# tambetm/simple_dqn

Hardware: AMD Instinct MI355X
Metric: train_steps/sec (batch=32, 4x84x84 uint8) (higher is better)
Workload: dtype f32; 1 GPU; BASELINE.json configs[1]: Breakout shapes, batch_size=32, replay_size=1000000, num_actions=4, HIP Q-net + device replay gather fused into conv1; global_batch=32, parallelism=dp1 (independent learners, RCCL grad all-reduce), ring=HBM mirror

## Files before the change

### __graft_entry__.py

```python
import os
import subprocess
import sys

ROOT = os.path.dirname(os.path.abspath(__file__))
if ROOT not in sys.path:
    sys.path.insert(0, ROOT)


def build():
    csrc = os.path.join(ROOT, "simple_dqn_amd", "csrc")
    subprocess.check_call(["make", "-C", csrc, "-j4"])
    emul = os.path.join(ROOT, "tests", "emul")
    subprocess.check_call(["g++", "-O2", "-ffp-contract=off", "-shared", "-fPIC", "-o", os.path.join(emul, "libsdqn_emul.so"),
                           os.path.join(emul, "emul.cpp")])
    subprocess.check_call(["g++", "-O2", "-ffp-contract=off", "-shared", "-fPIC", "-o", os.path.join(emul, "libsdqn_emul_n16.so"),
                           os.path.join(emul, "emul_n16.cpp")])
    from oracle import build_ref
    build_ref.build()
    import simple_dqn_amd
    lib = simple_dqn_amd.load()
    assert lib.sdqn_version() >= 100
    return None


def smoke():
    import random
    import numpy as np
    import simple_dqn_amd as sd
    sys.path.insert(0, os.path.join(ROOT, "tests"))
    from util import make_args
    from oracle.dqn_numpy import OracleDQN, xavier_weights
    from oracle.replay_numpy import ReplayOracle, synthetic_fill

    if not os.path.exists(sd.lib_path()):
        build()
    A, B, size = 4, 32, 2000
    args = make_args(batch_size=B)
    mem, omem = sd.ReplayMemory(size, args), ReplayOracle(size, batch_size=B)
    synthetic_fill(mem, 0, num_actions=A)
    synthetic_fill(omem, 0, num_actions=A)
    mem.sync_mirror()
    net = sd.DeepQNetwork(A, args)
    ws = xavier_weights(A, 1)
    net.set_weights(ws, 0)
    net.update_target_network()
    o = OracleDQN(A, batch_size=B, weights=ws)
    random.seed(3)
    mb = [x.copy() for x in mem.getMinibatch()]
    random.seed(3)
    omb = omem.getMinibatch()
    for a, b in zip(mb, omb):
        assert np.array_equal(a, b), "replay gather mismatch"
    random.seed(3)
    net.train_from_memory(mem, 1)
    o.train(omb)
    q, qo = net.predict(mb[0]), o.predict(omb[0])
    err = float(np.abs(q - qo).max())
    assert err < 1e-4, "Q-value mismatch vs oracle: %g" % err
    print("smoke ok: Q max-abs err vs oracle %.3e, gather bit-exact, B=%d" % (err, B))
    return None


if __name__ == "__main__":
    build()
    if len(sys.argv) > 1 and sys.argv[1] == "smoke":
        smoke()
```

### simple_dqn_amd/csrc/gemm_engine.h

```cpp
#pragma once
#include <hip/hip_runtime.h>
#include <string.h>
#include "problems.h"
#include "n16_map.h"
#include "launch.h"

namespace sdqn {

typedef float f32x16 __attribute__((ext_vector_type(16)));

template <class P, class = void> struct a_elem { typedef float type; };
template <class P> struct a_elem<P, decltype((void)sizeof(typename P::AT))> { typedef typename P::AT type; };
template <class P, class = void> struct b_elem { typedef float type; };
template <class P> struct b_elem<P, decltype((void)sizeof(typename P::BT))> { typedef typename P::BT type; };
template <class P, class = void> struct stages_lds { static constexpr bool value = false; };
template <class P> struct stages_lds<P, decltype((void)P::STAGE_LDS)> { static constexpr bool value = P::STAGE_LDS; };
template <class P> struct Staged : P { static constexpr bool STAGE_LDS = true; };
template <class P, class = void> struct a_group4 { static constexpr bool value = false; };
template <class P> struct a_group4<P, decltype((void)P::A_GROUP4)> { static constexpr bool value = P::A_GROUP4; };
template <class P, class = void> struct uses_f16_wgrad { static constexpr bool value = false; };
template <class P> struct uses_f16_wgrad<P, decltype((void)P::F16_WGRAD)> { static constexpr bool value = P::F16_WGRAD; };
template <class P, class = void> struct has_preload { static constexpr bool value = false; };
template <class P> struct has_preload<P, decltype((void)P::PRELOAD)> { static constexpr bool value = P::PRELOAD; };
template <class P, class = void> struct has_preload_multi { static constexpr bool value = false; };
template <class P> struct has_preload_multi<P, decltype((void)P::PRELOAD_MULTI)> { static constexpr bool value = P::PRELOAD_MULTI; };
struct Lead { const void* p[5]; int B, s0, s1, ctl, r0, r1; };
static_assert(sizeof(Lead) == 64, "leading block: 16 dwords");
constexpr int LEAD_ON = 256;
#define SDQN_LEAD_PARAMS const void* lp0, const void* lp1, const void* lp2, const void* lp3, const void* lp4, int lB, int ls0, int ls1, int lctl, int lr0, int lr1
#define SDQN_LEAD_ARGS(L) (L).p[0], (L).p[1], (L).p[2], (L).p[3], (L).p[4], (L).B, (L).s0, (L).s1, (L).ctl, (L).r0, (L).r1
template <class T> struct lead_noref { typedef T type; };
template <class T> struct lead_noref<T&> { typedef T type; };
#define SDQN_LEAD_SET_(f, v) a.f = (typename lead_noref<decltype(a.f)>::type)(v)
#define SDQN_LEAD_FIELDS(f0, f1, f2, f3, f4, X) \
  static void lead_pack(const StepArgs& a, Lead& l) { l.p[0] = a.f0; l.p[1] = a.f1; l.p[2] = a.f2; l.p[3] = a.f3; l.p[4] = a.f4; l.s1 = a.X; } \
  __device__ static void lead_apply(StepArgs& a, const void* q0, const void* q1, const void* q2, const void* q3, const void* q4, int x) { \
    SDQN_LEAD_SET_(f0, q0); SDQN_LEAD_SET_(f1, q1); SDQN_LEAD_SET_(f2, q2); SDQN_LEAD_SET_(f3, q3); SDQN_LEAD_SET_(f4, q4); a.X = x; }
template <class P, class = void> struct has_lead { static constexpr bool value = false; };
template <class P> struct has_lead<P, decltype((void)P::LEAD)> { static constexpr bool value = P::LEAD; };
template <class P, class = void> struct has_lead_multi { static constexpr bool value = false; };
template <class P> struct has_lead_multi<P, decltype((void)P::LEAD_MULTI)> { static constexpr bool value = P::LEAD_MULTI; };
inline int lead_grid(const dim3& g) { return (int)(g.x | g.y << 16 | g.z << 24); }
inline bool lead_grid_fits(const dim3& g) { return g.x < 65536u && g.y < 256u && g.z < 128u; }
inline int lead_ctl(const StepArgs& a, bool on) {
  const bool fits = a.B < 128 && a.xcd_map >= 0 && a.xcd_map < 256 && a.nz >= 0 && a.nz < 16 && a.S4 >= 0 && a.S4 < 256;
  return (a.xcd_map & 255) | (on && fits ? LEAD_ON : 0) | ((a.nz & 15) << 12) | ((a.S4 & 255) << 16);
}
__device__ __forceinline__ void lead_scalars(StepArgs& a, int B, int ctl) { a.B = B; a.xcd_map = ctl & 255; a.nz = (ctl >> 12) & 15; a.S4 = (ctl >> 16) & 255; }
#define SDQN_LEAD_FWD lp0, lp1, lp2, lp3, lp4, lB, ls0, ls1, lctl, lr0, lr1
template <class P, class = void> struct uses_f16_mfma { static constexpr bool value = false; };
template <class P> struct uses_f16_mfma<P, decltype((void)P::F16_MFMA)> { static constexpr bool value = P::F16_MFMA; };
template <class P, class = void> struct n16_waves { static constexpr int value = 0; };
template <class P> struct n16_waves<P, decltype((void)P::N16_WAVES)> { static constexpr int value = P::N16_WAVES; };
template <class P, int NW> constexpr bool use_n16() {
  return NW > 1 && n16_waves<P>::value == NW && stages_lds<P>::value && !uses_f16_wgrad<P>::value && !uses_f16_mfma<P>::value;
}
template <class P, class = void> struct gated_store { static constexpr bool value = false; };
template <class P> struct gated_store<P, decltype((void)P::GATED)> { static constexpr bool value = P::GATED; };

constexpr int PANEL = 32 * 33;

__device__ __forceinline__ void wave_lds_sync() {
  __builtin_amdgcn_fence(__ATOMIC_RELEASE, "wavefront");
  __builtin_amdgcn_wave_barrier();
  __builtin_amdgcn_fence(__ATOMIC_ACQUIRE, "wavefront");
}


__device__ __forceinline__ int pick_half(int v, int s, bool hi) {
  const int lo = __builtin_amdgcn_readlane(v, s), up = __builtin_amdgcn_readlane(v, s + 4);
  return hi ? up : lo;
}
__device__ __forceinline__ int64_t pick_half(int64_t v, int s, bool hi) {
  const int i = s;
  const int l0 = __builtin_amdgcn_readlane((int)(v & 0xFFFFFFFF), i), l1 = __builtin_amdgcn_readlane((int)(v >> 32), i);
  const int u0 = __builtin_amdgcn_readlane((int)(v & 0xFFFFFFFF), i + 4), u1 = __builtin_amdgcn_readlane((int)(v >> 32), i + 4);
  const int64_t lo = ((int64_t)l1 << 32) | (uint32_t)l0, up = ((int64_t)u1 << 32) | (uint32_t)u0;
  return hi ? up : lo;
}

#ifdef SDQN_TIMING
__device__ unsigned long long* g_sdqn_dbg = nullptr;
#define SDQN_STAMP(ph) do { if (g_sdqn_dbg && threadIdx.x == 0) g_sdqn_dbg[((size_t)(blockIdx.x + gridDim.x * (blockIdx.y + gridDim.y * blockIdx.z)) * 8) + (ph)] = clock64(); } while (0)
__device__ unsigned long long* g_sdqn_wdbg = nullptr;
__device__ unsigned g_sdqn_wdbg_blocks = 0;
#define SDQN_WSTAMP_DECL unsigned long long wst_[4] = {0, 0, 0, 0}
#define SDQN_WSTAMP(ph) do { if (wst_[ph] == 0) wst_[ph] = clock64(); } while (0)
#define SDQN_WSTAMP_FLUSH do { unsigned long long* wd_ = g_sdqn_wdbg; if (wd_ && (threadIdx.x & 63) == 0) { \
  const size_t b_ = (size_t)(blockIdx.x + gridDim.x * (blockIdx.y + gridDim.y * blockIdx.z)); const unsigned nb_ = g_sdqn_wdbg_blocks; \
  if (b_ < nb_ && (threadIdx.x >> 6) < 16) { \
    for (int q_ = 0; q_ < 4; ++q_) wd_[(b_ * 16 + (threadIdx.x >> 6)) * 4 + q_] = wst_[q_]; \
    if (threadIdx.x == 0) { unsigned x_; asm volatile("s_getreg_b32 %0, hwreg(HW_REG_XCC_ID, 0, 4)" : "=s"(x_)); wd_[(size_t)nb_ * 64 + b_] = x_; } } } } while (0)
#else
#define SDQN_STAMP(ph) do {} while (0)
#define SDQN_WSTAMP_DECL do {} while (0)
#define SDQN_WSTAMP(ph) do {} while (0)
#define SDQN_WSTAMP_FLUSH do {} while (0)
#endif

template <class P, int NW>
constexpr int tile_lds() {
  return NW * PANEL * (stages_lds<P>::value && (P::A_K || P::B_K) ? ((P::A_K ? 1 : 0) + (P::B_K ? 1 : 0)) : 1);
}

__device__ __forceinline__ constexpr int kslot(int t, int h) { return 8 * (t >> 2) + 4 * h + (t & 3); }

template <class T>
__device__ __forceinline__ T ld_byte_off(const T* base, uint32_t byte_off) {
  return *reinterpret_cast<const T*>(reinterpret_cast<const char*>(base) + byte_off);
// ... 278 lines not shown
      pan_a[n16::pan_off(n16::PA, k, x)] = pra[j].x; pan_a[n16::pan_off(n16::PA, k + 1, x)] = pra[j].y;
      pan_a[n16::pan_off(n16::PA, k + 2, x)] = pra[j].z; pan_a[n16::pan_off(n16::PA, k + 3, x)] = pra[j].w;
    }
#pragma unroll
    for (int j = 0; j < 2; ++j) {
      const int x = n16::ld_x(lane, j), k = n16::ld_k(lane);
      pan_b[n16::pan_off(n16::PB, k, x)] = prb[j].x; pan_b[n16::pan_off(n16::PB, k + 1, x)] = prb[j].y;
      pan_b[n16::pan_off(n16::PB, k + 2, x)] = prb[j].z; pan_b[n16::pan_off(n16::PB, k + 3, x)] = prb[j].w;
    }
    if (kc + NW * 32 < kend) stage_load(kc + NW * 32);
    wave_lds_sync();
#pragma unroll
    for (int t = 0; t < 8; ++t) { fa0[t] = pan_a[n16::frag_a(lane, t, 0)]; fa1[t] = pan_a[n16::frag_a(lane, t, 1)]; fb[t] = pan_b[n16::frag_b(lane, t)]; }
    wave_lds_sync();
#ifdef SDQN_TIMING
    asm volatile("" :: "v"(fa0[0]), "v"(fa1[7]));
    SDQN_WSTAMP(2);
    asm volatile("" :: "v"(fb[0]), "v"(fb[7]));
    SDQN_WSTAMP(3);
    SDQN_STAMP(3);
#endif
#pragma unroll
    for (int t = 0; t < 8; ++t) {
      acc0 = __builtin_amdgcn_mfma_f32_16x16x4f32(fa0[t], fb[t], acc0, 0, 0, 0);
      acc1 = __builtin_amdgcn_mfma_f32_16x16x4f32(fa1[t], fb[t], acc1, 0, 0, 0);
    }
    kc += NW * 32;
  }

#ifdef SDQN_TIMING
  asm volatile("" :: "v"(acc0[0]), "v"(acc1[3]));
  SDQN_STAMP(4);
#endif
  if (wave < NW) {
    float* cw = smem + wave * n16::WAVE_LDS;
#pragma unroll
    for (int r = 0; r < 4; ++r) {
      cw[n16::comb_off(n16::acc_row(0, lane, r), n16::acc_col(lane))] = acc0[r];
      cw[n16::comb_off(n16::acc_row(1, lane, r), n16::acc_col(lane))] = acc1[r];
    }
  }
  __syncthreads();
  SDQN_STAMP(5);
  static_assert(NT >= n16::TM * n16::TN, "one thread per element of the tile");
  if (mine) {
    float v = smem[n16::comb_off(ml, nl)];
#pragma unroll
    for (int w = 1; w < NW; ++w) v += smem[w * n16::WAVE_LDS + n16::comb_off(ml, nl)];
    if constexpr (gated_store<P>::value) P::store_gated(a, z, ks, m0 + ml, n0 + nl, v, gate);
    else P::store(a, z, ks, m0 + ml, n0 + nl, v);
  }
  SDQN_STAMP(6);
  SDQN_WSTAMP_FLUSH;
}

template <class P, int NW, int NT>
__device__ __forceinline__ void gemm_tile_h(const StepArgs& a, int bx, int by, int bz, float* smem) {
  constexpr int WAVE_LDS = PANEL;
  typedef typename P::aoff_t aoff_t;
  const int lane = threadIdx.x & 63;
  const int wave = __builtin_amdgcn_readfirstlane(threadIdx.x >> 6);
  const int m0 = bx * 32, n0 = by * 32;
  int z, ks, kbeg, kend;
  P::ksplit(a, bz, z, ks, kbeg, kend);
  if (NW * 64 < NT && wave >= NW) kend = kbeg;
  const int M = P::M(a), N = P::N(a);
  const int i = lane & 31, h8 = (lane >> 5) * 8;
  const aoff_t arow = P::a_row(a, z, m0 + i < M ? m0 + i : M - 1);
  const int bcol = P::b_col(a, z, n0 + i < N ? n0 + i : N - 1);
  f32x16 acc;
#pragma unroll
  for (int r = 0; r < 16; ++r) acc[r] = 0.0f;
  for (int kc = kbeg + (wave < NW ? wave : 0) * 32; kc < kend; kc += NW * 32) {
    const half8 fa0 = P::a_load8(a, z, arow + P::a_col(a, z, kc + h8));
    const half8 fb0 = P::b_load8(a, z, bcol + P::b_row(a, z, kc + h8));
    const half8 fa1 = P::a_load8(a, z, arow + P::a_col(a, z, kc + 16 + h8));
    const half8 fb1 = P::b_load8(a, z, bcol + P::b_row(a, z, kc + 16 + h8));
    acc = __builtin_amdgcn_mfma_f32_32x32x16_f16(fa0, fb0, acc, 0, 0, 0);
    acc = __builtin_amdgcn_mfma_f32_32x32x16_f16(fa1, fb1, acc, 0, 0, 0);
  }
  if constexpr (NW > 1) {
    if (wave < NW) {
      float* cw = smem + wave * WAVE_LDS;
#pragma unroll
      for (int r = 0; r < 16; ++r) {
        const int row = (r & 3) + 8 * (r >> 2) + 4 * (lane >> 5);
        cw[row * 33 + (lane & 31)] = acc[r];
      }
    }
    __syncthreads();
    for (int e = threadIdx.x; e < 1024; e += NT) {
      const int ml = e >> 5, nl = e & 31;
      float v = smem[ml * 33 + nl];
#pragma unroll
      for (int w = 1; w < NW; ++w) v += smem[w * WAVE_LDS + ml * 33 + nl];
      if (m0 + ml < M && n0 + nl < N) P::store(a, z, ks, m0 + ml, n0 + nl, v);
    }
  } else {
#pragma unroll
    for (int r = 0; r < 16; ++r) {
      const int ml = (r & 3) + 8 * (r >> 2) + 4 * (lane >> 5), nl = lane & 31;
      if (m0 + ml < M && n0 + nl < N) P::store(a, z, ks, m0 + ml, n0 + nl, acc[r]);
    }
  }
}

// ... 67 lines not shown
    wave_lds_sync();
#pragma unroll
    for (int s = 0; s < 2; ++s) {
      half8 fa, fb;
#pragma unroll
      for (int j = 0; j < 8; ++j) fb[j] = sb[(16 * s + 8 * hb + j) * HW_PITCH + i];
      if constexpr (P::A_U8) {
#pragma unroll
        for (int g = 0; g < 2; ++g) {
          const int src = 16 * s + 4 * g;
          const int l0 = __builtin_amdgcn_readlane((int)(cv & 0xFFFFFFFF), src), l1 = __builtin_amdgcn_readlane((int)((int64_t)cv >> 32), src);
          const int u0 = __builtin_amdgcn_readlane((int)(cv & 0xFFFFFFFF), src + 8), u1 = __builtin_amdgcn_readlane((int)((int64_t)cv >> 32), src + 8);
          const int64_t lo = ((int64_t)l1 << 32) | (uint32_t)l0, up = ((int64_t)u1 << 32) | (uint32_t)u0;
          const int64_t c = hi ? up : lo;
          const bool ok = kcur + 16 * s + 8 * hb + 4 * g < kend;
          const f4 v = P::a_load_group4(a, z, arow_own + c);
          fa[4 * g] = ok ? (half_t)v.x : (half_t)0.0f; fa[4 * g + 1] = ok ? (half_t)v.y : (half_t)0.0f;
          fa[4 * g + 2] = ok ? (half_t)v.z : (half_t)0.0f; fa[4 * g + 3] = ok ? (half_t)v.w : (half_t)0.0f;
        }
      } else {
#pragma unroll
        for (int j = 0; j < 8; ++j) fa[j] = sa[(16 * s + 8 * hb + j) * HW_PITCH + i];
      }
      acc = __builtin_amdgcn_mfma_f32_32x32x16_f16(fa, fb, acc, 0, 0, 0);
    }
    wave_lds_sync();
  }

  if constexpr (NW > 1) {
    if (wave < NW) {
      float* cw = smem + wave * HW_WAVE_LDS;
#pragma unroll
      for (int r = 0; r < 16; ++r) cw[((r & 3) + 8 * (r >> 2) + 4 * hb) * 33 + i] = acc[r];
    }
    __syncthreads();
    for (int e = threadIdx.x; e < 1024; e += NT) {
      const int ml = e >> 5, nl = e & 31;
      float v = smem[ml * 33 + nl];
#pragma unroll
      for (int w = 1; w < NW; ++w) v += smem[w * HW_WAVE_LDS + ml * 33 + nl];
      if (m0 + ml < M && n0 + nl < N) P::store(a, z, ks, m0 + ml, n0 + nl, v);
    }
  } else {
    float v[16];
#pragma unroll
    for (int r = 0; r < 16; ++r) v[r] = acc[r];
    P::store16(a, z, ks, m0, n0, lane, M, N, v, epi);
  }
}

template <class P, int NW, int NT>
__device__ __forceinline__ void run_tile(const StepArgs& a, int bx, int by, int bz, float* smem) {
  if constexpr (use_n16<P, NW>()) gemm_tile_n16<P, NW, NT>(a, bx, by, bz, smem);
  else if constexpr (uses_f16_wgrad<P>::value) gemm_tile_hw<P, NW, NT>(a, bx, by, bz, smem);
  else if constexpr (uses_f16_mfma<P>::value) gemm_tile_h<P, NW, NT>(a, bx, by, bz, smem);
  else gemm_tile<P, NW, NT>(a, bx, by, bz, smem);
}
template <class P, int NW>
constexpr int tile_lds_any() {
  if constexpr (use_n16<P, NW>()) return NW * n16::WAVE_LDS;
  else if constexpr (uses_f16_wgrad<P>::value) return NW * HW_WAVE_LDS;
  else return uses_f16_mfma<P>::value ? NW * PANEL : tile_lds<P, NW>();
}
template <class P> constexpr int tile_m() { return 32; }
template <class P, int NW = 0> constexpr int tile_n() { return use_n16<P, NW>() ? n16::TN : 32; }


template <class P>
__device__ __forceinline__ void lead_take(StepArgs& a, int& gx, int& gy, int& gz, const StepArgs& a_, SDQN_LEAD_PARAMS) {
  (void)lr0; (void)lr1;
  if (lctl & LEAD_ON) { lead_scalars(a, lB, lctl); P::lead_apply(a, lp0, lp1, lp2, lp3, lp4, ls1); gx = ls0 & 0xFFFF; gy = (ls0 >> 16) & 255; gz = ls0 >> 24; }
  else { if constexpr (has_preload<P>::value) P::preload(a_, gridDim.x, gridDim.y, gridDim.z); gx = gridDim.x; gy = gridDim.y; gz = gridDim.z; }
}
template <class P, int NW>
__device__ __forceinline__ void gemm_kernel_body(const StepArgs& a, int gx, int gy, int gz, float* smem) {
  const int lin = blockIdx.x + gx * (blockIdx.y + gy * blockIdx.z);
  const int t = (a.xcd_map & 1) ? xcd_tile_id(lin, gx * gy * gz) : lin;
  const int bz = t / (gx * gy), r = t - bz * (gx * gy);
  run_tile<P, NW, NW * 64>(a, r % gx, r / gx, bz, smem);
}
template <class P, int NW>
__global__ void __launch_bounds__(NW * 64) gemm_kernel(SDQN_LEAD_PARAMS, const StepArgs a_) {
  __shared__ float smem[tile_lds_any<P, NW>()];
  (void)lr0; (void)lr1;
  if constexpr (has_lead<P>::value) {
    StepArgs a = a_;
    int gx, gy, gz;
    lead_take<P>(a, gx, gy, gz, a_, SDQN_LEAD_FWD);
    gemm_kernel_body<P, NW>(a, gx, gy, gz, smem);
  } else {
    if constexpr (has_preload<P>::value) P::preload(a_, gridDim.x, gridDim.y, gridDim.z);
    gemm_kernel_body<P, NW>(a_, gridDim.x, gridDim.y, gridDim.z, smem);
  }
}

struct MultiDims { int n[3]; int gx[3], gy[3]; };

template <class P, int NW, int NT>
__device__ __forceinline__ void multi_dispatch(const StepArgs& a, const MultiDims& d, int which, int local, float* smem) {
  static_assert(!use_n16<P, NW>(), "multi-problem launches size their tile grids for 32 x 32 tiles");
  if constexpr (NW == 1) {
    const int wave = __builtin_amdgcn_readfirstlane(threadIdx.x >> 6);
    const int t = local * (NT / 64) + wave;
    const int per_z = d.gx[which] * d.gy[which];
    if (t < a.f4w_count) {
      const int tile = a.f4w_first + t;
      const int bz = tile / per_z, r = tile - bz * per_z;
      run_tile<P, 1, 64>(a, r % d.gx[which], r / d.gx[which], bz, smem);
    }
  } else {
    const int per_z = d.gx[which] * d.gy[which];
    const int bz = local / per_z, r = local - bz * per_z;
    run_tile<P, NW, NT>(a, r % d.gx[which], r / d.gx[which], bz, smem);
  }
}

template <int NT, class P0, int NW0, class P1, int NW1, class P2, int NW2>
__device__ __forceinline__ void gemm_multi_body(const StepArgs& a, const MultiDims& d, float* smem) {
  const int b = blockIdx.x;
  const int xm = a.xcd_map;
  if (b < d.n[0]) multi_dispatch<P0, NW0, NT>(a, d, 0, (xm & 1) ? xcd_tile_id_range(b, 0, d.n[0]) : b, smem);
  else if (b < d.n[0] + d.n[1]) multi_dispatch<P1, NW1, NT>(a, d, 1, (xm & 2) ? xcd_tile_id_range(b, d.n[0], d.n[1]) : b - d.n[0], smem);
  else multi_dispatch<P2, NW2, NT>(a, d, 2, (xm & 4) ? xcd_tile_id_range(b, d.n[0] + d.n[1], d.n[2]) : b - d.n[0] - d.n[1], smem);
}
template <int NT, class P0, int NW0, class P1, int NW1, class P2, int NW2>
__global__ void __launch_bounds__(NT) gemm_multi_kernel(SDQN_LEAD_PARAMS, const StepArgs a_, const MultiDims d_) {
  constexpr int L0 = tile_lds_any<P0, NW0>() * (NW0 == 1 ? NT / 64 : 1), L1 = tile_lds_any<P1, NW1>() * (NW1 == 1 ? NT / 64 : 1),
                L2 = tile_lds_any<P2, NW2>() * (NW2 == 1 ? NT / 64 : 1);
  constexpr int L = L0 > L1 ? (L0 > L2 ? L0 : L2) : (L1 > L2 ? L1 : L2);
  __shared__ float smem[L];
  (void)lr0; (void)lr1;
  if constexpr (has_lead_multi<P1>::value) {
    StepArgs a = a_; MultiDims d = d_;
    if (lctl & LEAD_ON) {
      lead_scalars(a, lB, lctl); P1::lead_apply(a, lp0, lp1, lp2, lp3, lp4, ls1);
      d.n[0] = ls0 & 0xFFFF; d.n[1] = (int)((unsigned)ls0 >> 16);
      d.gx[0] = (P0::M(a) + tile_m<P0>() - 1) / tile_m<P0>(); d.gy[0] = (P0::N(a) + tile_n<P0>() - 1) / tile_n<P0>();
      d.gx[1] = (P1::M(a) + tile_m<P1>() - 1) / tile_m<P1>(); d.gy[1] = (P1::N(a) + tile_n<P1>() - 1) / tile_n<P1>();
      d.gx[2] = (P2::M(a) + tile_m<P2>() - 1) / tile_m<P2>(); d.gy[2] = (P2::N(a) + tile_n<P2>() - 1) / tile_n<P2>();
    } else { if constexpr (has_preload_multi<P1>::value) P1::preload_multi(a_, d_); }
    gemm_multi_body<NT, P0, NW0, P1, NW1, P2, NW2>(a, d, smem);
  } else {
    if constexpr (has_preload_multi<P1>::value) P1::preload_multi(a_, d_);
    gemm_multi_body<NT, P0, NW0, P1, NW1, P2, NW2>(a_, d_, smem);
  }
}

struct NoProblem {
  static constexpr bool A_K = false, B_K = false; typedef int aoff_t; struct Epi {};
  static constexpr bool A_REG = false, A_U8 = false, B_REG = false; static constexpr int A_LD = 0, B_LD = 0;
  SDQN_HD static const float* a_ptr(const StepArgs&, int) { return nullptr; }
  SDQN_HD static const float* b_ptr(const StepArgs&, int) { return nullptr; }
  SDQN_HD static int M(const StepArgs&) { return 0; }
  SDQN_HD static int N(const StepArgs&) { return 0; }
  SDQN_HD static int nbz(const StepArgs&) { return 0; }
  SDQN_HD static void ksplit(const StepArgs&, int, int& z, int& ks, int& kb, int& ke) { z = ks = kb = ke = 0; }
  SDQN_HD static int a_row(const StepArgs&, int, int) { return 0; }
  SDQN_HD static int a_col(const StepArgs&, int, int) { return 0; }
  SDQN_HD static float a_load(const StepArgs&, int, int) { return 0.f; }
  SDQN_HD static f4 a_load4(const StepArgs&, int, int) { f4 o; o.x = o.y = o.z = o.w = 0.f; return o; }
  SDQN_HD static f4 b_load4(const StepArgs&, int, int) { f4 o; o.x = o.y = o.z = o.w = 0.f; return o; }
  SDQN_HD static int b_row(const StepArgs&, int, int) { return 0; }
  SDQN_HD static int b_col(const StepArgs&, int, int) { return 0; }
  SDQN_HD static float b_load(const StepArgs&, int, int) { return 0.f; }
  SDQN_HD static void store(const StepArgs&, int, int, int, int, float) {}
  __device__ static void epi_begin(const StepArgs&, int, int, int, Epi&) {}
  __device__ static void store16(const StepArgs&, int, int, int, int, int, int, int, const float*, Epi&) {}
};

template <class P, int NW>
inline hipError_t launch_gemm(const StepArgs& a, hipStream_t stream) {
  dim3 grid((P::M(a) + tile_m<P>() - 1) / tile_m<P>(), (P::N(a) + tile_n<P, NW>() - 1) / tile_n<P, NW>(), P::nbz(a));
  Lead l; memset(&l, 0, sizeof l);
  if constexpr (has_lead<P>::value) {
    P::lead_pack(a, l); l.B = a.B; l.s0 = lead_grid(grid);
    l.ctl = lead_ctl(a, a.arg_preload && lead_grid_fits(grid));
  }
  SDQN_LAUNCH((gemm_kernel<P, NW>), grid, dim3(NW * 64), 0, stream, SDQN_LEAD_ARGS(l), a);
  return hipGetLastError();
}

template <int NT, class P, int NW>
inline void multi_fill(const StepArgs& a, MultiDims& d, int i) {
  d.gx[i] = (P::M(a) + tile_m<P>() - 1) / tile_m<P>(); d.gy[i] = (P::N(a) + tile_n<P>() - 1) / tile_n<P>();
  const int tiles = d.gx[i] * d.gy[i] * P::nbz(a);
  d.n[i] = NW == 1 ? (a.f4w_count + NT / 64 - 1) / (NT / 64) : tiles;
}
template <int NT, class P0, int NW0, class P1, int NW1, class P2, int NW2>
inline hipError_t launch_multi(const StepArgs& a, bool has1, bool has2, hipStream_t stream) {
  static_assert(NW0 * 64 <= NT && NW1 * 64 <= NT && NW2 * 64 <= NT, "waves per tile exceed the workgroup");
  MultiDims d; memset(&d, 0, sizeof d);
  multi_fill<NT, P0, NW0>(a, d, 0);
  if (has1) multi_fill<NT, P1, NW1>(a, d, 1);
  if (has2) multi_fill<NT, P2, NW2>(a, d, 2);
  if (d.n[0] + d.n[1] + d.n[2] == 0) return hipSuccess;
  Lead l; memset(&l, 0, sizeof l);
  if constexpr (has_lead_multi<P1>::value) {
    P1::lead_pack(a, l); l.B = a.B; l.s0 = (int)((unsigned)d.n[0] | (unsigned)d.n[1] << 16);
    l.ctl = lead_ctl(a, a.arg_preload && has1 && has2 && d.n[0] < 65536 && d.n[1] < 65536);
  }
  SDQN_LAUNCH((gemm_multi_kernel<NT, P0, NW0, P1, NW1, P2, NW2>), dim3(d.n[0] + d.n[1] + d.n[2]), dim3(NT), 0, stream, SDQN_LEAD_ARGS(l), a, d);
  return hipGetLastError();
}

}
```

### simple_dqn_amd/csrc/problems.h

```cpp
#pragma once
#include <stddef.h>
#include <stdint.h>
#include <math.h>

#if defined(__HIPCC__)
#define SDQN_HD __host__ __device__ inline
#else
#define SDQN_HD inline
#endif

namespace sdqn {

constexpr int H0 = 84, W0 = 84, C0 = 4;
constexpr int FRAME = H0 * W0;
constexpr int STATE = C0 * FRAME;
constexpr int ST1 = 4, P1 = 20, Q1 = 20, K1 = 32;
constexpr int ST2 = 2, P2 = 9, Q2 = 9, K2 = 64;
constexpr int P3 = 7, Q3 = 7, K3 = 64;
constexpr int PIX1 = P1 * Q1, PIX2 = P2 * Q2, PIX3 = P3 * Q3;
constexpr int CRS1 = 256, CRS2 = 512, CRS3 = 576;
constexpr int NFC = 512, NIN4 = PIX3 * K3;
constexpr int PD3 = 11, PD2 = 11;
constexpr int NW1 = CRS1 * K1, NW2 = CRS2 * K2, NW3 = CRS3 * K3, NW4 = NIN4 * NFC;
constexpr int OFF1 = 0, OFF2 = OFF1 + NW1, OFF3 = OFF2 + NW2, OFF4 = OFF3 + NW3, OFF5 = OFF4 + NW4;
// ... 192 lines not shown
}


SDQN_HD int64_t row1(const StepArgs& a, int z, int m) {
  int n = m / PIX1, pix = m - n * PIX1, p = pix / Q1, q = pix - p * Q1;
  return sbase(a, z, n) + (int64_t)(p * ST1) * W0 + q * ST1;
}
SDQN_HD int col1(int k) { int c = k >> 6, r = (k >> 3) & 7, s = k & 7; return c * FRAME + r * W0 + s; }
SDQN_HD int row2(const StepArgs& a, int z, int m) {
  int n = m / PIX2, pix = m - n * PIX2, p = pix / Q2, q = pix - p * Q2;
  return (((z * a.B + n) * P1 + p * ST2) * Q1 + q * ST2) * K1;
}
SDQN_HD int col2(int k) { int r = k >> 7, s = (k >> 5) & 3, c = k & 31; return (r * Q1 + s) * K1 + c; }
SDQN_HD int row3(const StepArgs& a, int z, int m) {
  int n = m / PIX3, pix = m - n * PIX3, p = pix / Q3, q = pix - p * Q3;
  return (((z * a.B + n) * P2 + p) * Q2 + q) * K2;
}
SDQN_HD int col3(int k) { int rs = k >> 6, c = k & 63, r = rs / 3, s = rs - r * 3; return (r * Q2 + s) * K2 + c; }
SDQN_HD int prow2(int m) {
  int n = m / PIX2, pix = m - n * PIX2, p = pix / Q2, q = pix - p * Q2;
  return ((n * PD2 + p + 1) * PD2 + q + 1) * K2;
}

struct Conv1Fwd {
  static constexpr bool A_K = true, B_K = false;
  typedef int64_t aoff_t;
  static constexpr bool A_REG = false, A_U8 = true, B_REG = true; static constexpr int A_LD = 0, B_LD = K1;
  SDQN_HD static const float* a_ptr(const StepArgs& a, int z) { (void)z; return (const float*)nullptr; }
  SDQN_HD static const float* b_ptr(const StepArgs& a, int z) { (void)z; return a.theta[wslot(z)] + OFF1; }
#if defined(__HIPCC__)
  struct Epi {};
  __device__ static void epi_begin(const StepArgs&, int, int, int, Epi&) {}
  __device__ static void store16(const StepArgs& a, int z, int ks, int m0, int n0, int lane, int M, int N, const float* v, Epi&);
#endif
  SDQN_HD static int M(const StepArgs& a) { return a.B * PIX1; }
  SDQN_HD static int N(const StepArgs&) { return K1; }
  SDQN_HD static int nbz(const StepArgs& a) { return a.nz; }
  SDQN_HD static void ksplit(const StepArgs&, int bz, int& z, int& ks, int& kb, int& ke) { z = bz; ks = 0; kb = 0; ke = CRS1; }
  SDQN_HD static aoff_t a_row(const StepArgs& a, int z, int m) { return row1(a, z, m); }
  SDQN_HD static aoff_t a_col(const StepArgs&, int, int k) { return col1(k); }
  SDQN_HD static float a_load(const StepArgs& a, int, aoff_t o) { return norm_u8(a.src[o]); }
  SDQN_HD static f4 a_load4(const StepArgs& a, int, aoff_t o) { return ld4_u8(a.src + o); }
  SDQN_HD static int b_row(const StepArgs&, int, int k) { return k * K1; }
  SDQN_HD static int b_col(const StepArgs&, int, int n) { return n; }
  SDQN_HD static float b_load(const StepArgs& a, int z, int o) { return a.theta[wslot(z)][OFF1 + o]; }
  SDQN_HD static f4 b_load4(const StepArgs& a, int z, int o) { return ld4(a.theta[wslot(z)] + OFF1 + o); }
  SDQN_HD static void store(const StepArgs& a, int z, int, int m, int n, float v) {
    a.a1[((int64_t)z * M(a) + m) * K1 + n] = fmaxf(v, 0.0f);
  }
};

struct Conv2Fwd {
  static constexpr bool A_K = true, B_K = false;
  typedef int aoff_t;
  static constexpr bool A_REG = false, A_U8 = false, B_REG = true; static constexpr int A_LD = 0, B_LD = K2;
  SDQN_HD static const float* a_ptr(const StepArgs& a, int z) { (void)z; return a.a1; }
  SDQN_HD static const float* b_ptr(const StepArgs& a, int z) { (void)z; return a.theta[wslot(z)] + OFF2; }
#if defined(__HIPCC__)
  struct Epi {};
  __device__ static void epi_begin(const StepArgs&, int, int, int, Epi&) {}
  __device__ static void store16(const StepArgs& a, int z, int ks, int m0, int n0, int lane, int M, int N, const float* v, Epi&);
#endif
  SDQN_HD static int M(const StepArgs& a) { return a.B * PIX2; }
  SDQN_HD static int N(const StepArgs&) { return K2; }
  SDQN_HD static int nbz(const StepArgs& a) { return a.nz; }
  SDQN_HD static void ksplit(const StepArgs&, int bz, int& z, int& ks, int& kb, int& ke) { z = bz; ks = 0; kb = 0; ke = CRS2; }
  SDQN_HD static aoff_t a_row(const StepArgs& a, int z, int m) { return row2(a, z, m); }
  SDQN_HD static aoff_t a_col(const StepArgs&, int, int k) { return col2(k); }
  SDQN_HD static float a_load(const StepArgs& a, int, aoff_t o) { return a.a1[o]; }
  SDQN_HD static f4 a_load4(const StepArgs& a, int, aoff_t o) { return ld4(a.a1 + o); }
  SDQN_HD static int b_row(const StepArgs&, int, int k) { return k * K2; }
  SDQN_HD static int b_col(const StepArgs&, int, int n) { return n; }
  SDQN_HD static float b_load(const StepArgs& a, int z, int o) { return a.theta[wslot(z)][OFF2 + o]; }
  SDQN_HD static f4 b_load4(const StepArgs& a, int z, int o) { return ld4(a.theta[wslot(z)] + OFF2 + o); }
  SDQN_HD static void store(const StepArgs& a, int z, int, int m, int n, float v) {
    a.a2[((int64_t)z * M(a) + m) * K2 + n] = fmaxf(v, 0.0f);
  }
};

struct Conv3Fwd {
  static constexpr bool A_K = true, B_K = false;
  typedef int aoff_t;
  static constexpr bool A_REG = false, A_U8 = false, B_REG = true; static constexpr int A_LD = 0, B_LD = K3;
  SDQN_HD static const float* a_ptr(const StepArgs& a, int z) { (void)z; return a.a2; }
  SDQN_HD static const float* b_ptr(const StepArgs& a, int z) { (void)z; return a.theta[wslot(z)] + OFF3; }
#if defined(__HIPCC__)
  struct Epi {};
  __device__ static void epi_begin(const StepArgs&, int, int, int, Epi&) {}
  __device__ static void store16(const StepArgs& a, int z, int ks, int m0, int n0, int lane, int M, int N, const float* v, Epi&);
#endif
  SDQN_HD static int M(const StepArgs& a) { return a.B * PIX3; }
  SDQN_HD static int N(const StepArgs&) { return K3; }
  SDQN_HD static int nbz(const StepArgs& a) { return a.nz; }
  SDQN_HD static void ksplit(const StepArgs&, int bz, int& z, int& ks, int& kb, int& ke) { z = bz; ks = 0; kb = 0; ke = CRS3; }
  SDQN_HD static aoff_t a_row(const StepArgs& a, int z, int m) { return row3(a, z, m); }
  SDQN_HD static aoff_t a_col(const StepArgs&, int, int k) { return col3(k); }
  SDQN_HD static float a_load(const StepArgs& a, int, aoff_t o) { return a.a2[o]; }
  SDQN_HD static f4 a_load4(const StepArgs& a, int, aoff_t o) { return ld4(a.a2 + o); }
  SDQN_HD static int b_row(const StepArgs&, int, int k) { return k * K3; }
  SDQN_HD static int b_col(const StepArgs&, int, int n) { return n; }
  SDQN_HD static float b_load(const StepArgs& a, int z, int o) { return a.theta[wslot(z)][OFF3 + o]; }
  SDQN_HD static f4 b_load4(const StepArgs& a, int z, int o) { return ld4(a.theta[wslot(z)] + OFF3 + o); }
  SDQN_HD static void store(const StepArgs& a, int z, int, int m, int n, float v) {
    a.a3[((int64_t)z * M(a) + m) * K3 + n] = fmaxf(v, 0.0f);
  }
};
// ... 265 lines not shown
struct Conv1Wgrad {
  static constexpr bool A_K = false, B_K = false;
  typedef int64_t aoff_t;
  static constexpr bool A_REG = false, A_U8 = true, B_REG = true; static constexpr int A_LD = 0, B_LD = K1;
  SDQN_HD static const float* a_ptr(const StepArgs& a, int z) { (void)z; return (const float*)nullptr; }
  SDQN_HD static const float* b_ptr(const StepArgs& a, int z) { (void)z; return a.d1; }
#if defined(__HIPCC__)
  struct Epi {};
  __device__ static void epi_begin(const StepArgs&, int, int, int, Epi&) {}
  __device__ static void store16(const StepArgs& a, int z, int ks, int m0, int n0, int lane, int M, int N, const float* v, Epi&);
#endif
  SDQN_HD static int Kt(const StepArgs& a) { return a.B * PIX1; }
  SDQN_HD static int M(const StepArgs&) { return CRS1; }
  SDQN_HD static int N(const StepArgs&) { return K1; }
  SDQN_HD static int nbz(const StepArgs& a) { return ceil_div(ceil_div(Kt(a), 32), a.tps1); }
  SDQN_HD static void ksplit(const StepArgs& a, int bz, int& z, int& ks, int& kb, int& ke) {
    z = 0; ks = bz; kb = bz * a.tps1 * 32; ke = kb + a.tps1 * 32; if (ke > Kt(a)) ke = Kt(a);
  }
  SDQN_HD static aoff_t a_row(const StepArgs&, int, int m) { return col1(m); }
  SDQN_HD static aoff_t a_col(const StepArgs& a, int, int k) { return row1(a, 0, k); }
  SDQN_HD static float a_load(const StepArgs& a, int, aoff_t o) { return norm_u8(a.src[o]); }
  SDQN_HD static f4 a_load4(const StepArgs& a, int, aoff_t o) { return ld4_u8(a.src + o); }
  static constexpr bool A_GROUP4 = true;
  SDQN_HD static f4 a_load_group4(const StepArgs& a, int, aoff_t o) { return ld4_u8_stride4(a.src + o); }
  SDQN_HD static int b_row(const StepArgs&, int, int k) { return k * K1; }
  SDQN_HD static int b_col(const StepArgs&, int, int n) { return n; }
  SDQN_HD static float b_load(const StepArgs& a, int, int o) { return a.d1[o]; }
  SDQN_HD static f4 b_load4(const StepArgs& a, int, int o) { return ld4(a.d1 + o); }
  SDQN_HD static void store(const StepArgs& a, int, int ks, int m, int n, float v) { a.slab1[(int64_t)ks * NW1 + m * K1 + n] = v; }
};

#if defined(__HIPCC__)
#define SDQN_STORE16_DEFAULT(P) __device__ inline void P::store16(const StepArgs& a, int z, int ks, int m0, int n0, int lane, int M, int N, const float* v, P::Epi&) { \
  _Pragma("unroll") for (int r = 0; r < 16; ++r) { const int ml = (r & 3) + 8 * (r >> 2) + 4 * (lane >> 5), nl = lane & 31; \
    if (m0 + ml < M && n0 + nl < N) P::store(a, z, ks, m0 + ml, n0 + nl, v[r]); } }
SDQN_STORE16_DEFAULT(Conv1Fwd)
SDQN_STORE16_DEFAULT(Conv2Fwd)
SDQN_STORE16_DEFAULT(Conv3Fwd)
SDQN_STORE16_DEFAULT(Fc4Fwd)
SDQN_STORE16_DEFAULT(Fc4Dgrad)
SDQN_STORE16_DEFAULT(Conv3Dgrad)
SDQN_STORE16_DEFAULT(Conv3Wgrad)
SDQN_STORE16_DEFAULT(Conv2Dgrad)
SDQN_STORE16_DEFAULT(Conv2Wgrad)
SDQN_STORE16_DEFAULT(Conv1Wgrad)
#endif

struct Conv1FwdRaw : Conv1Fwd {
  SDQN_HD static void store(const StepArgs& a, int z, int, int m, int n, float v) { a.a1[((int64_t)z * M(a) + m) * K1 + n] = v; }
#if defined(__HIPCC__)
  __device__ static void store16(const StepArgs& a, int z, int ks, int m0, int n0, int lane, int M, int N, const float* v, Epi&);
#endif
};
struct Conv2FwdRaw : Conv2Fwd {
  SDQN_HD static void store(const StepArgs& a, int z, int, int m, int n, float v) { a.a2[((int64_t)z * M(a) + m) * K2 + n] = v; }
#if defined(__HIPCC__)
  __device__ static void store16(const StepArgs& a, int z, int ks, int m0, int n0, int lane, int M, int N, const float* v, Epi&);
#endif
};
struct Conv3FwdRaw : Conv3Fwd {
  SDQN_HD static void store(const StepArgs& a, int z, int, int m, int n, float v) { a.a3[((int64_t)z * M(a) + m) * K3 + n] = v; }
#if defined(__HIPCC__)
  __device__ static void store16(const StepArgs& a, int z, int ks, int m0, int n0, int lane, int M, int N, const float* v, Epi&);
#endif
};
#if defined(__HIPCC__)
SDQN_STORE16_DEFAULT(Conv1FwdRaw)
SDQN_STORE16_DEFAULT(Conv2FwdRaw)
SDQN_STORE16_DEFAULT(Conv3FwdRaw)
#endif

inline int64_t neon_to_internal(int layer, int64_t row, int64_t col) {
  switch (layer) {
    case 0: return row * K1 + col;
    case 1: { int c = (int)(row / 16), rs = (int)(row % 16); return ((int64_t)rs * 32 + c) * K2 + col; }
    case 2: { int c = (int)(row / 9), rs = (int)(row % 9); return ((int64_t)rs * 64 + c) * K3 + col; }
    case 3: { int f = (int)(col / PIX3), pix = (int)(col % PIX3); return ((int64_t)pix * K3 + f) * NFC + row; }
    default: return row * NFC + col;
  }
}
inline void layer_dims(int layer, int A, int64_t& rows, int64_t& cols, int64_t& off) {
  switch (layer) {
    case 0: rows = CRS1; cols = K1; off = OFF1; break;
    case 1: rows = CRS2; cols = K2; off = OFF2; break;
    case 2: rows = CRS3; cols = K3; off = OFF3; break;
    case 3: rows = NFC; cols = NIN4; off = OFF4; break;
    default: rows = A; cols = NFC; off = OFF5; break;
  }
}

}
```

### simple_dqn_amd/csrc/sdqn_kernels.hip

```cpp
#include "gemm_engine.h"
#include "problems_h16.h"
#include "kernels.h"
#include "update_body.h"

namespace sdqn {

static const char* k_names[K_COUNT] = {
  "conv1_fwd(gather+norm+conv+relu)", "conv2_fwd", "conv3_fwd", "fc4_fwd(splitK)", "head(fc5+td+delta)",
  "fc4_dgrad", "fc4_wgrad", "conv3_dgrad", "conv3_wgrad", "conv2_dgrad", "conv2_wgrad",
  "conv1_wgrad", "update(reduce+fc5wgrad+rmsprop)", "rccl_allreduce", "replay_gather_u8", "prep(idx+meta)",
  "bwd3(conv3_dgrad+conv3_wgrad+fc4_wgrad)", "bwd2(conv2_dgrad+conv2_wgrad+fc4_wgrad)", "bwd1(conv1_wgrad+fc4_wgrad)",
  "batchnorm(layer fwd/bwd)", "reserved", "reserved", "reserved", "reserved",
  "wgrads(fc4+conv3+conv2)", "act(conv1..fc5, one state)", "catch_collect(lockstep)", "target_blend(polyak)"};
const char* kernel_name(int id) { return (id >= 0 && id < K_COUNT) ? k_names[id] : "?"; }
LaunchEvents& launch_events() { static thread_local LaunchEvents le; return le; }

template <class P>
static hipError_t launch_nw(int nw, const StepArgs& a, hipStream_t s) {
  switch (nw) {
    case 2: return launch_gemm<P, 2>(a, s);
    case 4: return launch_gemm<P, 4>(a, s);
    case 8: return launch_gemm<P, 8>(a, s);
    case 16: return launch_gemm<P, 16>(a, s);
    default: return hipErrorInvalidValue;
  }
}

hipError_t launch_kernel(int id, const StepArgs& a, const LaunchTune& t, hipStream_t s) {
  const Route r = resolve_route(id, route_key(a, t), t);
  switch (r.unit) {
    case U_NONE: return hipSuccess;
    case U_SS: return launch_ss(r, id, a, t, s);
    case U_BT: return launch_bt(r, id, a, t, s);
    case U_R3: return launch_r3(r, id, a, t, s);
    case U_EXT: return launch_ext(r, id, a, t, s);
    case U_LAT: return launch_lat(r, id, a, t, s);
  }
  return hipErrorInvalidValue;
}

hipError_t launch_lat(const Route& r, int id, const StepArgs& a, const LaunchTune&, hipStream_t s) {
  switch (r.form) {
    case LAT_BN: case LAT_BN_B128: {
      const bool b128 = r.form == LAT_BN_B128;
      switch (id) {
        case K_CONV1_FWD: return launch_gemm<Conv1FwdRaw, 8>(a, s);
        case K_CONV2_FWD: return b128 ? launch_gemm<Staged<Conv2FwdRaw>, 8>(a, s) : launch_gemm<Conv2FwdRaw, 16>(a, s);
        case K_CONV3_FWD: return b128 ? launch_gemm<Staged<Conv3FwdRaw>, 8>(a, s) : launch_gemm<Staged<Conv3FwdRaw>, 9>(a, s);
        default: return hipErrorInvalidValue;
      }
    }
    case LAT_NW2: case LAT_NW4: case LAT_NW8: case LAT_NW9: case LAT_NW16: {
      const int nw = r.form == LAT_NW2 ? 2 : r.form == LAT_NW4 ? 4 : r.form == LAT_NW8 ? 8 : r.form == LAT_NW9 ? 9 : 16;
      switch (id) {
        case K_CONV1_FWD: return launch_nw<Conv1Fwd>(nw, a, s);
        case K_CONV2_FWD: return launch_nw<Conv2Fwd>(nw, a, s);
        case K_CONV3_FWD: if (nw == 9) return launch_gemm<Staged<Conv3Fwd>, 9>(a, s); return launch_nw<Conv3Fwd>(nw, a, s);
        case K_FC4_FWD: return launch_nw<Fc4Fwd>(nw, a, s);
        case K_FC4_DGRAD: return launch_nw<Fc4Dgrad>(nw, a, s);
        case K_CONV3_DGRAD: return launch_nw<Conv3Dgrad>(nw, a, s);
        case K_CONV3_WGRAD: return launch_nw<Conv3Wgrad>(nw, a, s);
        case K_CONV2_DGRAD: return launch_nw<Conv2Dgrad>(nw, a, s);
        case K_CONV2_WGRAD: return launch_nw<Conv2Wgrad>(nw, a, s);
        case K_CONV1_WGRAD: return launch_nw<Conv1Wgrad>(nw, a, s);
        default: return hipErrorInvalidValue;
      }
    }
    case LAT_THROUGHPUT: case LAT_THROUGHPUT_F4W:
      switch (id) {
        case K_CONV1_FWD: return launch_gemm<Conv1Fwd, 8>(a, s);
        case K_CONV2_FWD: return launch_gemm<Staged<Conv2Fwd>, 8>(a, s);
        case K_CONV3_FWD: return launch_gemm<Staged<Conv3Fwd>, 8>(a, s);
        case K_FC4_FWD: return launch_gemm<Staged<Fc4Fwd>, 8>(a, s);
        case K_FC4_DGRAD: return launch_gemm<Staged<Fc4Dgrad>, 4>(a, s);
        case K_CONV3_DGRAD: return launch_gemm<Staged<Conv3Dgrad>, 8>(a, s);
        case K_CONV2_DGRAD: return launch_gemm<Staged<Conv2Dgrad>, 8>(a, s);
        case K_BWD3:
          if (r.form == LAT_THROUGHPUT_F4W) return launch_multi<512, Fc4Wgrad, 8, Staged<Conv3Dgrad>, 8, Conv3Wgrad, 8>(a, true, true, s);
          return launch_multi<512, NoProblem, 2, Staged<Conv3Dgrad>, 8, Conv3Wgrad, 8>(a, true, true, s);
        case K_BWD2: return launch_multi<512, NoProblem, 2, Staged<Conv2Dgrad>, 8, Conv2Wgrad, 8>(a, true, true, s);
        default: return hipErrorInvalidValue;
      }
    case LAT_DEFAULT: case LAT_DEFAULT_F4W: case LAT_DEFAULT_B32_F4W: case LAT_F4W_NW1: case LAT_F4W_NW2: case LAT_F4W_NW4: case LAT_F4W_NW8: {
      const bool f4w = r.form == LAT_DEFAULT_F4W, b32 = r.form == LAT_DEFAULT_B32_F4W;
      switch (id) {
        case K_CONV1_FWD: return launch_gemm<Conv1Fwd, 8>(a, s);
        case K_CONV2_FWD: return launch_gemm<Conv2Fwd, 16>(a, s);
        case K_CONV3_FWD: return launch_gemm<Conv3Fwd, 16>(a, s);
        case K_FC4_FWD: return launch_gemm<Staged<Fc4Fwd>, 14>(a, s);
        case K_FC4_DGRAD:
          if (a.bn) return launch_gemm<Staged<Fc4DgradWide>, 16>(a, s);
          return launch_gemm<Staged<Fc4Dgrad>, 16>(a, s);
        case K_FC4_WGRAD:
          if (r.form == LAT_F4W_NW1) return launch_gemm<Fc4Wgrad, 1>(a, s);
          if (r.form == LAT_F4W_NW2) return launch_gemm<Fc4Wgrad, 2>(a, s);
          if (r.form == LAT_F4W_NW4) return launch_gemm<Fc4Wgrad, 4>(a, s);
          return launch_gemm<Fc4Wgrad, 8>(a, s);
        case K_CONV3_DGRAD: return launch_gemm<Staged<Conv3Dgrad>, 8>(a, s);
        case K_CONV3_WGRAD: return launch_gemm<Conv3Wgrad, 8>(a, s);
        case K_CONV2_DGRAD: return launch_gemm<Conv2Dgrad, 8>(a, s);
        case K_CONV2_WGRAD: return launch_gemm<Conv2Wgrad, 8>(a, s);
        case K_CONV1_WGRAD: return launch_gemm<Conv1Wgrad, 16>(a, s);
        case K_BWD3:
          if (b32) return launch_multi<512, Staged<Conv3Dgrad>, 8, Conv3Wgrad, 8, Fc4Wgrad, 1>(a, true, true, s);
          if (f4w) return launch_multi<512, Fc4Wgrad, 8, Staged<Conv3Dgrad>, 8, Conv3Wgrad, 8>(a, true, true, s);
          return launch_multi<512, NoProblem, 2, Staged<Conv3Dgrad>, 8, Conv3Wgrad, 8>(a, true, true, s);
        case K_BWD2:
          if (b32) return launch_multi<512, Fc4Wgrad, 1, Conv2Dgrad, 8, Conv2Wgrad, 8>(a, true, true, s);
          return launch_multi<512, NoProblem, 2, Conv2Dgrad, 8, Conv2Wgrad, 8>(a, true, true, s);
// ... 343 lines not shown
```

Measured before the change: 16180 train_steps/sec.

## Add 48x32 split-K tile body for conv2 forward with 16-wave LDS combine

Adds a new GEMM tile variant (48 rows by 32 columns) used when a problem declares M48_WAVES matching the wave count and is not LDS-staged. Conv2Fwd opts in at 16 waves, so the unstaged 16-wave conv2 forward launch now uses fewer, taller tiles. Each wave handles a strided k-slice, and partial sums are reduced through LDS in two halves of 8 waves. The aim is to cut tile count and reuse B loads across three row groups, at the cost of more LDS, extra barriers and possible padding waste when M is not a multiple of 48. The latency NW routes are redirected to a Wide alias that keeps the old path.

```diff
diff --git a/__graft_entry__.py b/__graft_entry__.py
--- a/__graft_entry__.py
+++ b/__graft_entry__.py
@@ -15,6 +15,8 @@
                            os.path.join(emul, "emul.cpp")])
     subprocess.check_call(["g++", "-O2", "-ffp-contract=off", "-shared", "-fPIC", "-o", os.path.join(emul, "libsdqn_emul_n16.so"),
                            os.path.join(emul, "emul_n16.cpp")])
+    subprocess.check_call(["g++", "-O2", "-ffp-contract=off", "-shared", "-fPIC", "-o", os.path.join(emul, "libsdqn_emul_m48.so"),
+                           os.path.join(emul, "emul_m48.cpp")])
     from oracle import build_ref
     build_ref.build()
     import simple_dqn_amd
diff --git a/simple_dqn_amd/csrc/gemm_engine.h b/simple_dqn_amd/csrc/gemm_engine.h
--- a/simple_dqn_amd/csrc/gemm_engine.h
+++ b/simple_dqn_amd/csrc/gemm_engine.h
@@ -3,6 +3,7 @@
 #include <string.h>
 #include "problems.h"
 #include "n16_map.h"
+#include "m48_map.h"
 #include "launch.h"
 
 namespace sdqn {
@@ -55,6 +56,11 @@
 template <class P, int NW> constexpr bool use_n16() {
   return NW > 1 && n16_waves<P>::value == NW && stages_lds<P>::value && !uses_f16_wgrad<P>::value && !uses_f16_mfma<P>::value;
 }
+template <class P, class = void> struct m48_waves { static constexpr int value = 0; };
+template <class P> struct m48_waves<P, decltype((void)P::M48_WAVES)> { static constexpr int value = P::M48_WAVES; };
+template <class P, int NW> constexpr bool use_m48() {
+  return NW > 1 && m48_waves<P>::value == NW && !stages_lds<P>::value && !uses_f16_wgrad<P>::value && !uses_f16_mfma<P>::value;
+}
 template <class P, class = void> struct gated_store { static constexpr bool value = false; };
 template <class P> struct gated_store<P, decltype((void)P::GATED)> { static constexpr bool value = P::GATED; };
 
@@ -439,6 +445,112 @@
   }
   SDQN_STAMP(6);
   SDQN_WSTAMP_FLUSH;
+}
+
+template <class P, int NW, int NT>
+__device__ __forceinline__ void gemm_tile_m48(const StepArgs& a, int bx, int by, int bz, float* smem) {
+  static_assert(P::A_K && !P::B_K && P::B_REG && !P::A_U8, "48 x 32 body: A k-contiguous floats, B a plain [k][n] matrix");
+  static_assert(NW == 2 * m48::HALF_WAVES && NT == NW * 64, "two combine halves of 8 waves, no surplus waves");
+  static_assert(sizeof(typename a_elem<P>::type) == 4 && sizeof(typename b_elem<P>::type) == 4, "fp32 operands");
+  typedef typename P::aoff_t aoff_t;
+  SDQN_STAMP(0);
+  const int lane = threadIdx.x & 63;
+  const int wave = __builtin_amdgcn_readfirstlane(threadIdx.x >> 6);
+  const int m0 = bx * m48::TM, n0 = by * m48::TN;
+  int z, ks, kbeg, kend;
+  P::ksplit(a, bz, z, ks, kbeg, kend);
+  const int M = P::M(a), N = P::N(a);
+  const float* bbase = P::b_ptr(a, z);
+  aoff_t srow[m48::RG][2]; int bcol[m48::CH];
+#pragma unroll
+  for (int rg = 0; rg < m48::RG; ++rg)
+#pragma unroll
+    for (int j = 0; j < 2; ++j) { const int m = m0 + m48::ld_row(lane, rg, j); srow[rg][j] = P::a_row(a, z, m < M ? m : M - 1); }
+#pragma unroll
+  for (int h = 0; h < m48::CH; ++h) { const int n = n0 + m48::frag_col(lane, h); bcol[h] = P::b_col(a, z, n < N ? n : N - 1); }
+  const int klane = m48::kslot_lane(lane >> 4);
+  float* pan = smem + m48::opnd_off(wave);
+
+  f32x4 acc[m48::RG][m48::CH];
+#pragma unroll
+  for (int rg = 0; rg < m48::RG; ++rg)
+#pragma unroll
+    for (int h = 0; h < m48::CH; ++h) acc[rg][h] = f32x4{0.0f, 0.0f, 0.0f, 0.0f};
+  SDQN_STAMP(1);
+  SDQN_STAMP(2);
+  for (int kc = kbeg + wave * 32; kc < kend; kc += NW * 32) {
+    f4 pra[m48::RG][2]; float fb[m48::CH][m48::STEPS];
+    const aoff_t c = P::a_col(a, z, kc + n16::ld_k(lane));
+#pragma unroll
+    for (int rg = 0; rg < m48::RG - 1; ++rg)
+#pragma unroll
+      for (int j = 0; j < 2; ++j) pra[rg][j] = P::a_load4(a, z, srow[rg][j] + c);
+#pragma unroll
+    for (int t = 0; t < m48::STEPS; ++t) {
+      const int r = P::b_row(a, z, kc + m48::kslot_step(t) + klane);
+#pragma unroll
+      for (int h = 0; h < m48::CH; ++h) fb[h][t] = bbase[(uint32_t)(r + bcol[h])];
+    }
+#ifdef SDQN_TIMING
+    asm volatile("" :: "v"(pra[0][0].x), "v"(pra[1][1].w), "v"(fb[0][0]), "v"(fb[1][7]));
+    SDQN_STAMP(3);
+#endif
+#pragma unroll
+    for (int rg = 0; rg < m48::RG; ++rg) {
+      float fa[m48::STEPS];
+#pragma unroll
+      for (int j = 0; j < 2; ++j) {
+        const int x = n16::ld_x(lane, j), k = n16::ld_k(lane);
+        pan[m48::pan_off(k, x)] = pra[rg][j].x; pan[m48::pan_off(k + 1, x)] = pra[rg][j].y;
+        pan[m48::pan_off(k + 2, x)] = pra[rg][j].z; pan[m48::pan_off(k + 3, x)] = pra[rg][j].w;
+      }
+      if (rg == 0) {
+#pragma unroll
+        for (int j = 0; j < 2; ++j) pra[m48::RG - 1][j] = P::a_load4(a, z, srow[m48::RG - 1][j] + c);
+      }
+      wave_lds_sync();
+#pragma unroll
+      for (int t = 0; t < m48::STEPS; ++t) fa[t] = pan[m48::frag_a(lane, t)];
+      wave_lds_sync();
+#pragma unroll
+      for (int t = 0; t < m48::STEPS; ++t)
+#pragma unroll
+        for (int h = 0; h < m48::CH; ++h) acc[rg][h] = __builtin_amdgcn_mfma_f32_16x16x4f32(fa[t], fb[h][t], acc[rg][h], 0, 0, 0);
+    }
+  }
+
+#ifdef SDQN_TIMING
+  asm volatile("" :: "v"(acc[0][0][0]), "v"(acc[2][1][3]));
+  SDQN_STAMP(4);
+#endif
+  const int e0 = threadIdx.x, e1 = threadIdx.x + NT;
+  const bool two = e1 < m48::TM * m48::TN;
+  const int o0 = m48::comb_off(m48::epi_row(e0), m48::epi_col(e0)), o1 = two ? m48::comb_off(m48::epi_row(e1), m48::epi_col(e1)) : o0;
+  float v0 = 0.0f, v1 = 0.0f;
+#pragma unroll
+  for (int half = 0; half < 2; ++half) {
+    if (half) __syncthreads();
+    if (m48::comb_half(wave) == half) {
+      float* cw = smem + m48::comb_panel(wave) * m48::PANEL_C;
+#pragma unroll
+      for (int rg = 0; rg < m48::RG; ++rg)
+#pragma unroll
+        for (int h = 0; h < m48::CH; ++h)
+#pragma unroll
+          for (int r = 0; r < 4; ++r) cw[m48::comb_off(m48::acc_row(rg, lane, r), m48::acc_col(h, lane))] = acc[rg][h][r];
+    }
+    __syncthreads();
+    if (half) SDQN_STAMP(5);
+#pragma unroll
+    for (int w = 0; w < m48::HALF_WAVES; ++w) {
+      const float p0 = smem[w * m48::PANEL_C + o0];
+      v0 = (half == 0 && w == 0) ? p0 : v0 + p0;
+      if (two) { const float p1 = smem[w * m48::PANEL_C + o1]; v1 = (half == 0 && w == 0) ? p1 : v1 + p1; }
+    }
+  }
+  { const int m = m0 + m48::epi_row(e0), n = n0 + m48::epi_col(e0); if (m < M && n < N) P::store(a, z, ks, m, n, v0); }
+  if (two) { const int m = m0 + m48::epi_row(e1), n = n0 + m48::epi_col(e1); if (m < M && n < N) P::store(a, z, ks, m, n, v1); }
+  SDQN_STAMP(6);
 }
 
 template <class P, int NW, int NT>
@@ -612,6 +724,7 @@
 template <class P, int NW, int NT>
 __device__ __forceinline__ void run_tile(const StepArgs& a, int bx, int by, int bz, float* smem) {
   if constexpr (use_n16<P, NW>()) gemm_tile_n16<P, NW, NT>(a, bx, by, bz, smem);
+  else if constexpr (use_m48<P, NW>()) gemm_tile_m48<P, NW, NT>(a, bx, by, bz, smem);
   else if constexpr (uses_f16_wgrad<P>::value) gemm_tile_hw<P, NW, NT>(a, bx, by, bz, smem);
   else if constexpr (uses_f16_mfma<P>::value) gemm_tile_h<P, NW, NT>(a, bx, by, bz, smem);
   else gemm_tile<P, NW, NT>(a, bx, by, bz, smem);
@@ -619,10 +732,11 @@
 template <class P, int NW>
 constexpr int tile_lds_any() {
   if constexpr (use_n16<P, NW>()) return NW * n16::WAVE_LDS;
+  else if constexpr (use_m48<P, NW>()) return m48::LDS_FLOATS;
   else if constexpr (uses_f16_wgrad<P>::value) return NW * HW_WAVE_LDS;
   else return uses_f16_mfma<P>::value ? NW * PANEL : tile_lds<P, NW>();
 }
-template <class P> constexpr int tile_m() { return 32; }
+template <class P, int NW = 0> constexpr int tile_m() { return use_m48<P, NW>() ? m48::TM : 32; }
 template <class P, int NW = 0> constexpr int tile_n() { return use_n16<P, NW>() ? n16::TN : 32; }
 
 
@@ -658,7 +772,7 @@
 
 template <class P, int NW, int NT>
 __device__ __forceinline__ void multi_dispatch(const StepArgs& a, const MultiDims& d, int which, int local, float* smem) {
-  static_assert(!use_n16<P, NW>(), "multi-problem launches size their tile grids for 32 x 32 tiles");
+  static_assert(!use_n16<P, NW>() && !use_m48<P, NW>(), "multi-problem launches size their tile grids for 32 x 32 tiles");
   if constexpr (NW == 1) {
     const int wave = __builtin_amdgcn_readfirstlane(threadIdx.x >> 6);
     const int t = local * (NT / 64) + wave;
@@ -730,7 +844,7 @@
 
 template <class P, int NW>
 inline hipError_t launch_gemm(const StepArgs& a, hipStream_t stream) {
-  dim3 grid((P::M(a) + tile_m<P>() - 1) / tile_m<P>(), (P::N(a) + tile_n<P, NW>() - 1) / tile_n<P, NW>(), P::nbz(a));
+  dim3 grid((P::M(a) + tile_m<P, NW>() - 1) / tile_m<P, NW>(), (P::N(a) + tile_n<P, NW>() - 1) / tile_n<P, NW>(), P::nbz(a));
   Lead l; memset(&l, 0, sizeof l);
   if constexpr (has_lead<P>::value) {
     P::lead_pack(a, l); l.B = a.B; l.s0 = lead_grid(grid);
diff --git a/simple_dqn_amd/csrc/m48_map.h b/simple_dqn_amd/csrc/m48_map.h
--- /dev/null
+++ b/simple_dqn_amd/csrc/m48_map.h
@@ -0,0 +1,39 @@
+#pragma once
+#include "n16_map.h"
+
+namespace sdqn {
+namespace m48 {
+
+constexpr int TM = 48, TN = 32, KC = 32;
+constexpr int RG = TM / 16, CH = TN / 16;
+constexpr int STEPS = KC / 4;
+constexpr int PC = 36;
+constexpr int PANEL_C = TM * PC;
+constexpr int HALF_WAVES = 8;
+
+SDQN_HD constexpr int kslot_step(int t) { return n16::kslot(t, 0); }
+SDQN_HD constexpr int kslot_lane(int g) { return n16::kslot(0, g); }
+constexpr bool kslot_splits() {
+  for (int t = 0; t < STEPS; ++t) for (int g = 0; g < 4; ++g) if (n16::kslot(t, g) != kslot_step(t) + kslot_lane(g)) return false;
+  return true;
+}
+static_assert(kslot_splits(), "the k-slot map is a step part plus a lane part");
+constexpr int PANEL_A = n16::PANEL_B;
+SDQN_HD constexpr int ld_row(int lane, int rg, int j) { return 16 * rg + n16::ld_x(lane, j); }
+SDQN_HD constexpr int pan_off(int k, int x) { return n16::pan_off(n16::PB, k, x); }
+SDQN_HD constexpr int frag_a(int lane, int t) { return n16::frag_b(lane, t); }
+SDQN_HD constexpr int frag_row(int lane, int rg) { return 16 * rg + (lane & 15); }
+SDQN_HD constexpr int frag_col(int lane, int h) { return 16 * h + (lane & 15); }
+SDQN_HD constexpr int acc_row(int rg, int lane, int r) { return 16 * rg + 4 * (lane >> 4) + r; }
+SDQN_HD constexpr int acc_col(int h, int lane) { return 16 * h + (lane & 15); }
+SDQN_HD constexpr int comb_off(int row, int col) { return row * PC + col; }
+SDQN_HD constexpr int comb_half(int wave) { return wave / HALF_WAVES; }
+SDQN_HD constexpr int comb_panel(int wave) { return wave % HALF_WAVES; }
+SDQN_HD constexpr int opnd_off(int wave) { return wave < HALF_WAVES ? wave * PANEL_C : HALF_WAVES * PANEL_C + (wave - HALF_WAVES) * PANEL_A; }
+constexpr int LDS_FLOATS = HALF_WAVES * PANEL_C + HALF_WAVES * PANEL_A;
+static_assert(PANEL_A <= PANEL_C && LDS_FLOATS * 4 <= 80 * 1024, "A panels inside the owner's combine panel; the launch keeps to 80 KB");
+SDQN_HD constexpr int epi_row(int e) { return e >> 5; }
+SDQN_HD constexpr int epi_col(int e) { return e & 31; }
+
+}
+}
diff --git a/simple_dqn_amd/csrc/problems.h b/simple_dqn_amd/csrc/problems.h
--- a/simple_dqn_amd/csrc/problems.h
+++ b/simple_dqn_amd/csrc/problems.h
@@ -268,6 +268,7 @@
 
 struct Conv2Fwd {
   static constexpr bool A_K = true, B_K = false;
+  static constexpr int M48_WAVES = 16;
   typedef int aoff_t;
   static constexpr bool A_REG = false, A_U8 = false, B_REG = true; static constexpr int A_LD = 0, B_LD = K2;
   SDQN_HD static const float* a_ptr(const StepArgs& a, int z) { (void)z; return a.a1; }
@@ -639,7 +640,9 @@
   __device__ static void store16(const StepArgs& a, int z, int ks, int m0, int n0, int lane, int M, int N, const float* v, Epi&);
 #endif
 };
+struct Conv2FwdWide : Conv2Fwd { static constexpr int M48_WAVES = 0; };
 struct Conv2FwdRaw : Conv2Fwd {
+  static constexpr int M48_WAVES = 0;
   SDQN_HD static void store(const StepArgs& a, int z, int, int m, int n, float v) { a.a2[((int64_t)z * M(a) + m) * K2 + n] = v; }
 #if defined(__HIPCC__)
   __device__ static void store16(const StepArgs& a, int z, int ks, int m0, int n0, int lane, int M, int N, const float* v, Epi&);
diff --git a/simple_dqn_amd/csrc/sdqn_kernels.hip b/simple_dqn_amd/csrc/sdqn_kernels.hip
--- a/simple_dqn_amd/csrc/sdqn_kernels.hip
+++ b/simple_dqn_amd/csrc/sdqn_kernels.hip
@@ -54,7 +54,7 @@
       const int nw = r.form == LAT_NW2 ? 2 : r.form == LAT_NW4 ? 4 : r.form == LAT_NW8 ? 8 : r.form == LAT_NW9 ? 9 : 16;
       switch (id) {
         case K_CONV1_FWD: return launch_nw<Conv1Fwd>(nw, a, s);
-        case K_CONV2_FWD: return launch_nw<Conv2Fwd>(nw, a, s);
+        case K_CONV2_FWD: return launch_nw<Conv2FwdWide>(nw, a, s);
         case K_CONV3_FWD: if (nw == 9) return launch_gemm<Staged<Conv3Fwd>, 9>(a, s); return launch_nw<Conv3Fwd>(nw, a, s);
         case K_FC4_FWD: return launch_nw<Fc4Fwd>(nw, a, s);
         case K_FC4_DGRAD: return launch_nw<Fc4Dgrad>(nw, a, s);
```

After: 16380 train_steps/sec (median of 6 runs). 1.01x the previous value.
